# lean-dojo/ReProver

Hardware: AMD Instinct MI355X
Metric: retrieve QPS@top-100 (state encode + masked similarity top-k), ByT5-small, 130k-premise corpus (higher is better)
Workload: dtype bf16; 1 GPU; configs[1]: ByT5-small encode+retrieve, 130k premises, batch=256 states/GPU, top-100, bf16; n_premises=130000, states_per_gpu=256, k=100, state_len_mix=clip(round(LogNormal(ln 180, 0.9)), 16, 2048) bytes, index=row-sharded 1-way, bf16 unit-norm random rows, weights=random-init ByT5-small (d_model 1472, 12 layers, 6 heads, d_ff 3584)

## Files before the change

reprover_amd/csrc/rp_encoder.hip:

```cpp
#include <limits.h>

#include "rp_encoder_kernels.h"

namespace rp {

thread_local std::string g_last_error;

int g_gemm_group_m = 8;
constexpr int GEMM_VARIANT_BIG = 26, GEMM_VARIANT_O_BY_SIZE = -1;
int g_gemm_variant = GEMM_VARIANT_BIG;
int g_gemm_variant_qkv = GEMM_VARIANT_BIG;
int g_gemm_variant_wo = GEMM_VARIANT_BIG;
int g_gemm_variant_o = GEMM_VARIANT_O_BY_SIZE;
int g_gemm_small_pipe = 1;
int g_gemm_helpers = 64;
int g_gemm_persist = 9;
int g_pool_chunk = 64;
int g_gemm_edge_layout = 1;
int g_gemm_mixed = 20;
int g_gemm_mixed_bwd = 1;
int g_debug_skip_ffn = 0;
int g_gemm_skinny = 1;
int g_gemm_skinny_variant = 0;
int g_gemm_stagger_us[RP_K_COUNT] = {};

struct ProfRec {
  int cls;
  hipEvent_t a, b;
};
static bool g_prof_on = false;
static std::vector<ProfRec> g_prof_recs;
static std::vector<hipEvent_t> g_prof_pool;

static hipEvent_t prof_event() {
  if (!g_prof_pool.empty()) {
    hipEvent_t e = g_prof_pool.back();
    g_prof_pool.pop_back();
    return e;
  }
  hipEvent_t e;
  (void)hipEventCreate(&e);
  return e;
}
void prof_begin(hipStream_t stream, int kernel_class) {
  if (!g_prof_on) return;
  ProfRec r{kernel_class, prof_event(), prof_event()};
  (void)hipEventRecord(r.a, stream);
  g_prof_recs.push_back(r);
}
void prof_end(hipStream_t stream) {
  if (!g_prof_on) return;
  (void)hipEventRecord(g_prof_recs.back().b, stream);
}

}


using namespace rp;

extern "C" int32_t rp_abi_version(void) { return 7; }
extern "C" const char* rp_last_error(void) { return g_last_error.c_str(); }

namespace {
enum OptKind { OPT_PLAIN, OPT_BOOL };
struct Option {
  const char* name;
  int* var;
  int lo, hi;
  OptKind kind;
  bool (*valid)(int);
};
constexpr int ANY_LO = INT_MIN, ANY_HI = INT_MAX;
const Option g_options[] = {
    {"gemm_group_m", &g_gemm_group_m, 1, 64, OPT_PLAIN, nullptr},
    {"gemm_variant", &g_gemm_variant, ANY_LO, ANY_HI, OPT_PLAIN, gemm_variant_known},
    {"gemm_variant_qkv", &g_gemm_variant_qkv, ANY_LO, ANY_HI, OPT_PLAIN, gemm_variant_known},
    {"gemm_variant_wo", &g_gemm_variant_wo, ANY_LO, ANY_HI, OPT_PLAIN, gemm_variant_known},
    {"gemm_variant_o", &g_gemm_variant_o, ANY_LO, ANY_HI, OPT_PLAIN, gemm_variant_known},
    {"debug_skip_ffn", &g_debug_skip_ffn, ANY_LO, ANY_HI, OPT_BOOL, nullptr},
    {"gemm_skinny_variant", &g_gemm_skinny_variant, 0, 15, OPT_PLAIN, [](int v) { return v == 0 || v == 15; }},
    {"gemm_small_pipe", &g_gemm_small_pipe, ANY_LO, ANY_HI, OPT_BOOL, nullptr},
    {"pool_chunk", &g_pool_chunk, 32, 128, OPT_PLAIN, [](int v) { return v == 32 || v == 64 || v == 128; }},
    {"gemm_persist", &g_gemm_persist, ANY_LO, ANY_HI, OPT_PLAIN, nullptr},
    {"gemm_edge_layout", &g_gemm_edge_layout, ANY_LO, ANY_HI, OPT_BOOL, nullptr},
    {"gemm_mixed", &g_gemm_mixed, 0, 31, OPT_PLAIN, nullptr},
    {"gemm_mixed_bwd", &g_gemm_mixed_bwd, ANY_LO, ANY_HI, OPT_BOOL, nullptr},
    {"gemm_skinny", &g_gemm_skinny, ANY_LO, ANY_HI, OPT_BOOL, nullptr},
    {"scan_cfg", &g_scan_cfg, 0, 1, OPT_PLAIN, nullptr},
#ifdef RP_EXPERIMENTS
    {"scan_filter_cfg", &g_scan_filter_cfg, ANY_LO, ANY_HI, OPT_PLAIN, nullptr},
    {"scan_sample_cfg", &g_scan_sample_cfg, ANY_LO, ANY_HI, OPT_PLAIN, nullptr},
    {"scan_waves", &g_scan_waves, ANY_LO, ANY_HI, OPT_PLAIN, nullptr},
    {"scan_stride", &g_scan_stride, ANY_LO, ANY_HI, OPT_PLAIN, nullptr},
    {"train_dbg", &g_train_dbg, ANY_LO, ANY_HI, OPT_PLAIN, nullptr},
    {"scan_no_epilogue", &g_scan_no_epilogue, ANY_LO, ANY_HI, OPT_PLAIN, nullptr},
#endif
    {"train_wgrad_form", &g_train_wgrad_form, 0, 3, OPT_PLAIN, nullptr},
    {"scan_cap", &g_scan_cap, ANY_LO, ANY_HI, OPT_PLAIN, nullptr},
    {"scan_force_new", &g_scan_impl_force_new, ANY_LO, ANY_HI, OPT_PLAIN, nullptr},
    {"scan_small_tiles", &g_scan_small_tiles, 0, 1, OPT_PLAIN, nullptr},
    {"scan_impl", &g_scan_impl, 0, 1, OPT_PLAIN, nullptr},
};
}

extern "C" RpStatus rp_set_option(const char* name, int32_t value) {
  if (!strcmp(name, "gemm_variant_all")) {
    RP_REQUIRE(value == -1 || gemm_variant_known(value), "gemm_variant_all: tile configuration %d is not in this build", value);
    g_gemm_variant = g_gemm_variant_qkv = g_gemm_variant_wo = value < 0 ? GEMM_VARIANT_BIG : value;
    g_gemm_variant_o = value < 0 ? GEMM_VARIANT_O_BY_SIZE : value;
    return RP_OK;
  }
  if (!strcmp(name, "gemm_helpers")) {
    RP_REQUIRE(value >= 0 && value <= 248, "gemm_helpers out of range");
    g_gemm_helpers = value & ~7;
    return RP_OK;
  }
#ifdef RP_EXPERIMENTS
  if (!strncmp(name, "gemm_stagger_us_", 16)) {
    const char* which = name + 16;
    const int cls = !strcmp(which, "qkv") ? RP_K_GEMM_QKV : !strcmp(which, "o") ? RP_K_GEMM_O
                    : !strcmp(which, "wi") ? RP_K_GEMM_WI : !strcmp(which, "wo") ? RP_K_GEMM_WO : -1;
    RP_REQUIRE(cls >= 0 && value >= 0 && value <= 1000, "gemm_stagger_us: unknown GEMM or value out of range");
    g_gemm_stagger_us[cls] = value;
    return RP_OK;
  }
#endif
  for (const Option& o : g_options) {
    if (strcmp(name, o.name)) continue;
    RP_REQUIRE(value >= o.lo && value <= o.hi, "%s out of range", o.name);
    RP_REQUIRE(!o.valid || o.valid(value), "%s: %d is not one of its values in this build", o.name, value);
    *o.var = o.kind == OPT_BOOL ? value != 0 : value;
    return RP_OK;
  }
  return fail(RP_E_INVALID, "unknown option %s", name);
}

extern "C" RpStatus rp_profile_enable(int32_t on) {
  for (auto& r : g_prof_recs) {
    g_prof_pool.push_back(r.a);
    g_prof_pool.push_back(r.b);
  }
  g_prof_recs.clear();
// ... 201 lines not shown
    ProfScope ps(stream, RP_K_EMBED);
    auto launch_embed = [&](auto kern, int rows_per_wave) {
      hipLaunchKernelGGL(kern, dim3((Tp + 4 * rows_per_wave - 1) / (4 * rows_per_wave)), dim3(256), 0, stream, ids,
                         (const bf16_t*)e->embed_hi, (const uint8_t*)e->embed_lo, (const float*)e->embed_ss, w.xb,
                         reinterpret_cast<uint8_t*>(w.xlo), w.ssp, np, embed_rs ? w.rs : (float*)nullptr, 1.f / (float)D,
                         c.layer_norm_eps, T, Tp, D, c.vocab_size, t_dev);
    };
    const bool few = Tp < 8192;
    if (D <= 1536) {
      if (few) launch_embed(embed_copy_kernel<3, 1>, 1);
      else launch_embed(embed_copy_kernel<3, 4>, 4);
    } else {
      if (few) launch_embed(embed_copy_kernel<4, 1>, 1);
      else launch_embed(embed_copy_kernel<4, 4>, 4);
    }
  }
  RP_CHECK_LAUNCH();
  const dim3 att_grid(H, T / ATT_Q + batch);
  const int pc = g_pool_chunk;
  launch_worklist(cu_seqlens, batch, w.work, (int)att_grid.y, w.pwork, T / pc + batch, pc, stream);
  for (int i = 0; i < c.num_layers; ++i) {
    const LayerPacked& L = e->layers[i];
    if (!(i == 0 && embed_rs)) launch_rowscale();
    st = fused_rs ? launch_gemm<true>(w.xb, D, Tp, L.wqkv, D, 3 * inner, D,
                                      EpiStoreBf16Slots{w.qkv, 3 * inner, 3 * inner, rs_slots}, stream, RP_K_GEMM_QKV, tv, t_dev)
                  : launch_gemm(w.xb, D, Tp, L.wqkv, D, 3 * inner, D, EpiStoreBf16{w.qkv, 3 * inner, 3 * inner, rs}, stream,
                                RP_K_GEMM_QKV, tv, t_dev);
    if (st) return st;
    {
      ProfScope ps(stream, RP_K_ATTENTION);
      hipLaunchKernelGGL(attention_kernel<false>, att_grid, dim3(256), 0, stream, w.qkv, (const int4*)w.work, e->bias_tab, w.att,
                         H, e->maxd, (float*)nullptr, 0, Drop{0u, 0u, 1.f}, 0u);
    }
    if ((st = launch_gemm(w.att, inner, Tp, L.wo, inner, D, inner, EpiResid8{w.xb, w.xlo, D, D, w.ssp, np, Tp}, stream,
                          RP_K_GEMM_O, tv, t_dev)))
      return st;
    if (g_debug_skip_ffn) continue;
    launch_rowscale();
    st = fused_rs ? launch_gemm<true>(w.xb, D, Tp, L.wi, D, 2 * F, D, EpiGegluBf16Slots{w.ff, F, 2 * F, rs_slots}, stream,
                                      RP_K_GEMM_WI, tv, t_dev)
                  : launch_gemm(w.xb, D, Tp, L.wi, D, 2 * F, D, EpiGegluBf16{w.ff, F, 2 * F, rs}, stream, RP_K_GEMM_WI, tv,
                                t_dev);
    if (st) return st;
    if ((st = launch_gemm(w.ff, F, Tp, L.wo2, F, D, F, EpiResid8{w.xb, w.xlo, D, D, w.ssp, np, Tp}, stream, RP_K_GEMM_WO, tv,
                          t_dev)))
      return st;
  }
  launch_rowscale(true);
  if (hidden) {
    hipLaunchKernelGGL(hidden_out_kernel, dim3(T), dim3(256), 0, stream, w.xb, reinterpret_cast<const uint8_t*>(w.xlo), w.rs,
                       e->final_ln, hidden, D);
    RP_CHECK_LAUNCH();
    return RP_OK;
  }
  {
    ProfScope ps(stream, RP_K_POOL);
    launch_pool_partial(dim3(T / pc + batch), stream, w.xb, w.xlo, w.rs, (const int4*)w.pwork, w.pool, D, pc, e->final_ln, out,
                        out_dtype == RP_DT_BF16 ? 1 : 0, 1, true);
    launch_pool_finish(batch, stream, w.pool, e->final_ln, cu_seqlens, out, out_dtype == RP_DT_BF16 ? 1 : 0, D, pc, 1);
  }
  RP_CHECK_LAUNCH();
  return RP_OK;
}

extern "C" RpStatus rp_encode_hidden(RpEncoder* e, const int32_t* ids, const int32_t* cu_seqlens, int32_t batch, int32_t T,
                                     int32_t max_len, void* out, void* workspace, size_t workspace_bytes, void* stream_) {
  RP_REQUIRE(e && ids && cu_seqlens && out, "null argument");
  RP_REQUIRE(batch > 0 && T > 0 && max_len > 0 && max_len <= T, "batch=%d total_tokens=%d max_len=%d", batch, T,
             max_len);
  Workspace w = carve(e, T, batch, (char*)workspace);
  if (!workspace || workspace_bytes < w.bytes)
    return fail(RP_E_WORKSPACE, "workspace %zu < required %zu bytes", workspace_bytes, w.bytes);
  return encode_pass(e, ids, cu_seqlens, batch, T, nullptr, nullptr, RP_DT_BF16, w, (hipStream_t)stream_, (bf16_t*)out);
}

extern "C" RpStatus rp_encode_varlen(RpEncoder* e, const int32_t* ids, const int32_t* cu_seqlens, int32_t batch,
                                     int32_t T, int32_t max_len, void* out, int32_t out_dtype, void* workspace,
// ... 168 lines not shown
  PaddedPrep pp = carve_padded(batch, padded_len, (char*)workspace);
  Workspace w = carve(e, T_max, batch, workspace ? (char*)workspace + pp.bytes : nullptr);
  if (!workspace || workspace_bytes < pp.bytes + w.bytes)
    return fail(RP_E_WORKSPACE, "workspace %zu < required %zu bytes", workspace_bytes, pp.bytes + w.bytes);
  if (batch == 1) {
    hipLaunchKernelGGL(padded_single_kernel, dim3(1), dim3(1024), 0, stream, attention_mask, input_ids, padded_len, pp.lens,
                       pp.cu, pp.packed, meta);
  } else {
    hipLaunchKernelGGL(padded_lens_kernel, dim3(batch), dim3(256), 0, stream, attention_mask, padded_len, pp.lens);
    hipLaunchKernelGGL(padded_scan_kernel, dim3(1), dim3(1024), 0, stream, pp.lens, batch, pp.cu, meta);
    hipLaunchKernelGGL(padded_pack_kernel, dim3((padded_len + 255) / 256, batch), dim3(256), 0, stream, input_ids, pp.cu,
                       padded_len, pp.packed);
  }
  RP_CHECK_LAUNCH();
  return encode_pass(e, pp.packed, pp.cu, batch, T_max, meta , out, out_dtype, w, stream);
}

extern "C" RpStatus rp_dbg_gemm(const void* A, const void* W, void* out, int32_t M, int32_t N, int32_t K,
                                int32_t n_valid, int32_t epilogue, void* stream_) {
  hipStream_t stream = (hipStream_t)stream_;
  const bf16_t* a = (const bf16_t*)A;
  const bf16_t* w = (const bf16_t*)W;
  switch (epilogue) {
    case RP_EPI_STORE_BF16:
      return launch_gemm(a, K, M, w, K, N, K, EpiStoreBf16{(bf16_t*)out, n_valid, n_valid, RowScale{nullptr}}, stream,
                         RP_K_GEMM_QKV);
    case RP_EPI_RESID:
      RP_REQUIRE(n_valid % 8 == 0, "n_valid=%d", n_valid);
      return launch_gemm(a, K, M, w, K, N, K,
                         EpiResid{(bf16_t*)out, (bf16_t*)out + (size_t)M * n_valid, n_valid, n_valid, nullptr, 0, 0}, stream,
                         RP_K_GEMM_WO);
    case RP_EPI_RESID8:
      RP_REQUIRE(n_valid % 8 == 0, "n_valid=%d", n_valid);
      return launch_gemm(a, K, M, w, K, N, K,
                         EpiResid8{(bf16_t*)out, (bf16_t*)out + (size_t)M * n_valid, n_valid, n_valid, nullptr, 0, 0}, stream,
                         RP_K_GEMM_WO);
    case RP_EPI_GEGLU_BF16:
      return launch_gemm(a, K, M, w, K, N, K, EpiGegluBf16{(bf16_t*)out, n_valid / 2, n_valid, RowScale{nullptr}}, stream,
                         RP_K_GEMM_WI);
  }
  return fail(RP_E_INVALID, "unknown epilogue %d", epilogue);
}

extern "C" RpStatus rp_dbg_gemm_fused(const void* A, const void* W, void* out, int32_t M, int32_t N, int32_t K,
                                      int32_t n_valid, int32_t epilogue, const float* ssp_in, int32_t np_in,
                                      float inv_d, float eps, void* xb_out, float* ssp_out, int32_t np_out,
                                      void* stream_) {
  hipStream_t stream = (hipStream_t)stream_;
  const bf16_t* a = (const bf16_t*)A;
  const bf16_t* w = (const bf16_t*)W;
  float* rs_buf = nullptr;
  if (ssp_in) {
    RP_HIP(hipMalloc((void**)&rs_buf, (size_t)M * 4));
    hipLaunchKernelGGL(rowscale_kernel, dim3((M + 63) / 64), dim3(64), 0, stream, ssp_in, rs_buf, M, np_in, inv_d, eps);
  }
  const RowScale rs{rs_buf};
  struct Free {
    float* p;
    hipStream_t s;
    ~Free() {
      if (p) {
        (void)hipStreamSynchronize(s);
        (void)hipFree(p);
      }
    }
  } free_rs{rs_buf, stream};
  switch (epilogue) {
    case RP_EPI_STORE_BF16:
      return launch_gemm(a, K, M, w, K, N, K, EpiStoreBf16{(bf16_t*)out, n_valid, n_valid, rs}, stream, RP_K_GEMM_QKV);
    case RP_EPI_RESID:
      RP_REQUIRE(n_valid % 8 == 0, "n_valid=%d", n_valid);
      return launch_gemm(a, K, M, w, K, N, K,
                         EpiResid{(bf16_t*)out, (bf16_t*)out + (size_t)M * n_valid, n_valid, n_valid, ssp_out, np_out, M},
                         stream, RP_K_GEMM_WO);
    case RP_EPI_RESID8:
      RP_REQUIRE(n_valid % 8 == 0, "n_valid=%d", n_valid);
      return launch_gemm(a, K, M, w, K, N, K,
                         EpiResid8{(bf16_t*)out, (bf16_t*)out + (size_t)M * n_valid, n_valid, n_valid, ssp_out, np_out, M},
                         stream, RP_K_GEMM_WO);
    case RP_EPI_GEGLU_BF16:
      return launch_gemm(a, K, M, w, K, N, K, EpiGegluBf16{(bf16_t*)out, n_valid / 2, n_valid, rs}, stream,
                         RP_K_GEMM_WI);
  }
  return fail(RP_E_INVALID, "unknown epilogue %d", epilogue);
}

namespace rp {
__global__ __launch_bounds__(256) void mfma_probe_kernel(int mfmas, float* __restrict__ sink) {
  const uint32_t seed = (uint32_t)(blockIdx.x * 256 + threadIdx.x) * 2654435761u + 12345u;
  bf16x8 a[4], b[4];
#pragma unroll
  for (int i = 0; i < 4; ++i)
#pragma unroll
    for (int e = 0; e < 8; ++e) {
      const uint32_t h = (seed + 40503u * (uint32_t)(i * 8 + e)) * 2246822519u;
      a[i][e] = (short)(0x3f00 | (h & 0x80ff) | ((h >> 9) & 0x0080));
      b[i][e] = (short)(0x3f00 | ((h >> 16) & 0x80ff) | ((h >> 3) & 0x0080));
    }
  f32x16 acc[8];
#pragma unroll
  for (int i = 0; i < 8; ++i)
#pragma unroll
    for (int r = 0; r < 16; ++r) acc[i][r] = 0.f;
  for (int it = 0; it < mfmas; it += 32) {
#pragma unroll
    for (int rot = 0; rot < 4; ++rot)
#pragma unroll
      for (int i = 0; i < 8; ++i) acc[i] = __builtin_amdgcn_mfma_f32_32x32x16_bf16(a[i & 3], b[(i + rot) & 3], acc[i], 0, 0, 0);
  }
  float s = 0.f;
// ... 44 lines not shown
```

reprover_amd/csrc/rp_encoder_kernels.h:

```cpp
#pragma once
#include <math.h>
#include <string.h>

#include <algorithm>
#include <functional>
#include <vector>

#include "rp_gemm.h"

namespace rp {

extern int g_gemm_group_m, g_gemm_variant, g_gemm_variant_qkv, g_gemm_variant_wo, g_gemm_variant_o, g_debug_skip_ffn, g_gemm_skinny,
    g_gemm_skinny_variant, g_gemm_small_pipe, g_gemm_helpers, g_gemm_persist, g_pool_chunk, g_gemm_edge_layout, g_gemm_mixed,
    g_gemm_mixed_bwd, g_scan_waves, g_scan_small_tiles, g_scan_cfg, g_scan_impl, g_scan_filter_cfg, g_scan_sample_cfg, g_scan_stride,
    g_scan_no_epilogue, g_scan_impl_force_new, g_scan_cap, g_train_dbg, g_train_wgrad_form;
extern int g_gemm_stagger_us[RP_K_COUNT];

template <typename T>
__device__ __forceinline__ float load_as_f32(const void* p, size_t i);
template <>
__device__ __forceinline__ float load_as_f32<float>(const void* p, size_t i) {
  return reinterpret_cast<const float*>(p)[i];
}
template <>
__device__ __forceinline__ float load_as_f32<bf16_t>(const void* p, size_t i) {
  return bf2f(reinterpret_cast<const bf16_t*>(p)[i]);
}

enum PackMode { PACK_CONCAT3 = 0, PACK_GEGLU = 1, PACK_COPY = 2 };

template <typename T>
__global__ void pack_rows_kernel(bf16_t* dst, const void* s0, const void* s1, const void* s2,
                                 int rows_dst, int cols, int n, int mode, const float* colscale) {
  const int r = blockIdx.x;
  const void* src;
  int sr;
  if (mode == PACK_CONCAT3) {
    src = (r < n) ? s0 : (r < 2 * n ? s1 : s2);
    sr = r % n;
  } else if (mode == PACK_GEGLU) {
    src = ((r >> 5) & 1) ? s1 : s0;
    sr = (r >> 6) * 32 + (r & 31);
  } else {
    src = s0;
    sr = r;
  }
// ... 236 lines not shown
    for (int j = 0; j < FN; ++j) scv[j] = rs.get(n_base + j * 32 + cl);
#pragma unroll
    for (int ih = 0; ih < FM; ih += 2) {
      const int f = m_base + ih * 32 + sub * 8;
#pragma unroll
      for (int jb = 0; jb < FN; jb += 2) {
#pragma unroll
        for (int jj = 0; jj < 2 && jb + jj < FN; ++jj) {
          const float sc = scv[jb + jj];
#pragma unroll
          for (int i = 0; i < 2; ++i)
#pragma unroll
            for (int g = 0; g < 4; ++g) {
              uint2 v;
              v.x = pack_bf2(acc[ih + i][jb + jj][4 * g] * sc, acc[ih + i][jb + jj][4 * g + 1] * sc);
              v.y = pack_bf2(acc[ih + i][jb + jj][4 * g + 2] * sc, acc[ih + i][jb + jj][4 * g + 3] * sc);
              *reinterpret_cast<uint2*>(stage + (jj * 32 + cl) * EPI_ROW_BYTES + (i * 32 + 8 * g + 4 * hi) * 2) = v;
            }
        }
        const int nrows = (FN - jb >= 2) ? 64 : 32;
#pragma unroll
        for (int t0 = 0; t0 < 64; t0 += RPI) {
          const int t = t0 + rr;
          if (t < nrows) {
            const uint4 v = *reinterpret_cast<const uint4*>(stage + t * EPI_ROW_BYTES + sub * 16);
            if (f < n_valid) *reinterpret_cast<uint4*>(out + (size_t)(n_base + jb * 32 + t) * ldo + f) = v;
          }
        }
      }
    }
  }
};

template <bool SPLIT_IN, bool LO8 = false>
struct EpiResidT {
  static constexpr bool any_layout = true;
  bf16_t* __restrict__ xhi;
  bf16_t* __restrict__ xlo;
  int ldx, n_valid;
  float* __restrict__ ssp;
  int np, ssp_ld;
  const bf16_t* __restrict__ xhi_in = nullptr;
  Drop drop = {0u, 0u, 1.f};
  uint32_t drop_site = 0;
  template <int FM, int FN>
  __device__ __forceinline__ void run(f32x16 (&acc)[FM][FN], int m_base, int n_base, int lane, char* stage) {
    static_assert(FM % 2 == 0, "one statistic slot per 64 features (two row fragments)");
    const int hi = lane >> 5, cl = lane & 31;
    const int sub = lane & 7, rr = lane >> 3;
    constexpr int RB = 272;
    constexpr int NB = (FM / 2) * FN;
    constexpr int DEPTH = (FM * FN >= 16) ? 4 : 2;
    uint4 xh[DEPTH][4];
    typename std::conditional<LO8, uint2, uint4>::type xl[DEPTH][4];
    const uint8_t* xlo8 = reinterpret_cast<const uint8_t*>(xlo);
    auto fetch = [&](int b, int p) {
      const int q = b / FN, j = b % FN;
      const int f = min(m_base + q * 64 + sub * 8, n_valid - 8);
#pragma unroll
      for (int c = 0; c < 4; ++c) {
        const size_t off = (size_t)(n_base + j * 32 + c * 8 + rr) * ldx + f;
#ifdef RP_ABL_NOLOAD
        RP_ABL_NOLOAD_BODY(xh[p][c], xl[p][c], off);
#else
        if constexpr (SPLIT_IN)
          xh[p][c] = *reinterpret_cast<const uint4*>(xhi_in + off);
        else
          xh[p][c] = *reinterpret_cast<const uint4*>(xhi + off);
        if constexpr (LO8)
          xl[p][c] = *reinterpret_cast<const uint2*>(xlo8 + off);
        else
          xl[p][c] = *reinterpret_cast<const uint4*>(xlo + off);
#endif
      }
    };
#pragma unroll
    for (int b = 0; b < DEPTH - 1 && b < NB; ++b) fetch(b, b);
#pragma unroll
    for (int b = 0; b < NB; ++b) {
      const int q = b / FN, j = b % FN;
      const int f = m_base + q * 64 + sub * 8;
      const int slot = (m_base >> 6) + q;
      if (b + DEPTH - 1 < NB) fetch(b + DEPTH - 1, (b + DEPTH - 1) % DEPTH);
#pragma unroll
      for (int i = 0; i < 2; ++i)
#pragma unroll
        for (int g = 0; g < 4; ++g)
          *reinterpret_cast<float4*>(stage + cl * RB + (i * 32 + 8 * g + 4 * hi) * 4) =
              make_float4(acc[2 * q + i][j][4 * g], acc[2 * q + i][j][4 * g + 1], acc[2 * q + i][j][4 * g + 2],
                          acc[2 * q + i][j][4 * g + 3]);
#pragma unroll
      for (int c = 0; c < 4; ++c) {
        const int t = c * 8 + rr;
        float4 d0 = *reinterpret_cast<const float4*>(stage + t * RB + sub * 32);
        float4 d1 = *reinterpret_cast<const float4*>(stage + t * RB + sub * 32 + 16);
        if constexpr (SPLIT_IN) {
          if (drop.thresh) {
            const uint32_t row = (uint32_t)(n_base + j * 32 + t), c0 = (uint32_t)f;
            float m[8];
#pragma unroll
            for (int e = 0; e < 8; e += 2) drop_mul2(drop, drop_site, row, c0 + e, m[e], m[e + 1]);
            d0.x *= m[0]; d0.y *= m[1]; d0.z *= m[2]; d0.w *= m[3];
            d1.x *= m[4]; d1.y *= m[5]; d1.z *= m[6]; d1.w *= m[7];
          }
        }
        float ss = 0.f;
        if (f < n_valid) {
          const size_t off = (size_t)(n_base + j * 32 + t) * ldx + f;
          const uint4 h = xh[b % DEPTH][c];
          const auto l = xl[b % DEPTH][c];
          uint4 oh;
          typename std::conditional<LO8, uint2, uint4>::type ol;
          if constexpr (LO8) {
            x24_update8(h, l, d0, d1, oh, ol, ss);
          } else {
            hilo_update2(h.x, l.x, d0.x, d0.y, oh.x, ol.x, ss);
            hilo_update2(h.y, l.y, d0.z, d0.w, oh.y, ol.y, ss);
            hilo_update2(h.z, l.z, d1.x, d1.y, oh.z, ol.z, ss);
            hilo_update2(h.w, l.w, d1.z, d1.w, oh.w, ol.w, ss);
          }
#ifdef RP_ABL_NOSTORE
          RP_ABL_KEEP6(oh.x, oh.y, oh.z, oh.w, ol.x, ol.y);
#else
          *reinterpret_cast<uint4*>(xhi + off) = oh;
          if constexpr (LO8)
            *reinterpret_cast<uint2*>(reinterpret_cast<uint8_t*>(xlo) + off) = ol;
          else
            *reinterpret_cast<uint4*>(xlo + off) = ol;
#endif
        }
        if (ssp) {
          ss += dpp_f32<0xB1>(ss);
          ss += dpp_f32<0x4E>(ss);
          ss += dpp_f32<0x141>(ss);
          if (sub == 0 && slot < np) ssp[(size_t)slot * ssp_ld + n_base + j * 32 + t] = ss;
        }
      }
    }
  }
};

typedef EpiResidT<false> EpiResid;
typedef EpiResidT<false, true> EpiResid8;

#ifndef RP_GEGLU_PRELOAD
#define RP_GEGLU_PRELOAD 1
#endif
template <class RS>
struct EpiGegluBf16T {
  using main_layout = WaveLayout<2, 4, 4, 2>;
  bf16_t* out;
  int ldo, n_valid;
  RS rs;
  static constexpr bool preload_hook = std::is_same<RS, RowScale>::value && RP_GEGLU_PRELOAD;
  float pre[4] = {0.f, 0.f, 0.f, 0.f};
  template <int FN>
  __device__ __forceinline__ void preload(int n_base, int lane) {
    static_assert(FN <= 4, "pre[]");
#pragma unroll
    for (int j = 0; j < FN; ++j) pre[j] = rs.get(n_base + j * 32 + (lane & 31));
  }
  template <int FM, int FN, bool PRE = false>
  __device__ __forceinline__ void run(f32x16 (&acc)[FM][FN], int m_base, int n_base, int lane, char* stage) {
    static_assert(FM % 2 == 0, "gate/up fragment pairs");
    const int hi = lane >> 5, cl = lane & 31;
    constexpr int LPR = FM * 2;
    constexpr int RPI = 64 / LPR;
    static_assert(FM * 32 <= 128, "staging row");
    const int sub = lane % LPR, rr = lane / LPR;
    const int f = (m_base >> 1) + sub * 8;
    float scv[FN];
#pragma unroll
    for (int j = 0; j < FN; ++j) {
      if constexpr (PRE)
        scv[j] = pre[j];
      else
// ... 890 lines not shown
```

reprover_amd/csrc/rp_gemm.h:

```cpp
#pragma once
#include <type_traits>
#include "rp_util.h"

namespace rp {

#ifdef RP_PHASE_PROBE
#include "probes/rp_probe_hooks.h"
#else
#define RP_TS(slot) ((void)0)
#define RP_TS_PLAIN(slot) ((void)0)
#define RP_HTS(kt, which) ((void)0)
#define RP_PROBE_STAGE_FILTER(kt, half) ((void)0)
#define RP_PROBE_READS_DECL ((void)0)
#define RP_PROBE_READS_GATE ((void)0)
#define RP_PROBE_READS_PRIME(read_frags, smem) ((void)0)
#define RP_PTS_DECL ((void)0)
#define RP_PTS(v) ((void)0)
#define RP_PROBE_PERSIST_TILE_END(more) ((void)0)
#endif

__device__ __forceinline__ int mfma32_row(int r, int hi) { return (r & 3) + 8 * (r >> 2) + 4 * hi; }

template <int BM_, int BN_, int BK_, int WM_, int WN_, int NSTAGE_, int PIPE_ = 0, int FP8_ = 0, int AAUX_ = 0, int KTAIL_ = 0,
          int OCC_ = 0>
// ... 17 lines not shown
  static constexpr int A_DMA = BM / ROWS_PER_DMA / NWAVES, W_DMA = BN / ROWS_PER_DMA / NWAVES;
  static_assert(BM % (ROWS_PER_DMA * NWAVES) == 0 && BN % (ROWS_PER_DMA * NWAVES) == 0, "DMA split");
  static_assert(BK == 32 || BK == 64, "BK");
  __device__ static __forceinline__ int swz(int row) { return (BK == 32) ? ((row >> 2) & 3) : ((row >> 1) & 7); }
  __device__ static __forceinline__ int off(int row, int kc) { return row * ROW_BYTES + ((kc ^ swz(row)) << 4); }
};

template <int WM_, int WN_, int FM_, int FN_>
struct WaveLayout {
  static constexpr int WM = WM_, WN = WN_, FM = FM_, FN = FN_;
};

constexpr int EPI_ROW_BYTES = 144;
constexpr int EPI_STAGE_BYTES = 64 * EPI_ROW_BYTES;

struct GemmOperand {
  const bf16_t* ptr;
  int ld;
  int rows;
  __device__ __forceinline__ size_t row_off(int r, int kc) const { return (size_t)min(r, rows - 1) * ld + kc * 8; }
  __device__ __forceinline__ size_t k_off(int kt, int BK) const { return (size_t)kt * BK; }
};

template <class E, class = void>
struct has_prologue : std::false_type {};
template <class E>
struct has_prologue<E, std::void_t<decltype(&E::prologue)>> : std::true_type {};

template <class E, class = void>
struct has_preload : std::false_type {};
template <class E>
struct has_preload<E, std::enable_if_t<E::preload_hook>> : std::true_type {};

typedef __attribute__((address_space(3))) void* lds_ptr_t;
typedef const __attribute__((address_space(1))) void* gbl_ptr_t;

template <int N>
__device__ __forceinline__ void wait_vmcnt() {
  asm volatile("s_waitcnt vmcnt(%0)" ::"n"(N) : "memory");
}

template <class C, class Epilogue>
__device__ __forceinline__ void gemm_tile(const GemmOperand A, const GemmOperand W, int K, int tile_m,
                                          int tile_n, Epilogue& epi, char* smem) {
  constexpr int BK = C::BK, NSTAGE = C::NSTAGE, FM = C::FM, FN = C::FN;
  RP_TS_PLAIN(0);
  const int tid = threadIdx.x;
  const int lane = tid & 63;
  const int wave = __builtin_amdgcn_readfirstlane(tid >> 6);
  const int wave_row = wave / C::WN, wave_col = wave % C::WN;
  const int hi = lane >> 5;

  f32x16 acc[FM][FN];
#pragma unroll
  for (int i = 0; i < FM; ++i)
#pragma unroll
    for (int j = 0; j < FN; ++j)
#pragma unroll
      for (int r = 0; r < 16; ++r) acc[i][j][r] = 0.f;

  const bf16_t* a_src[C::A_DMA];
  const bf16_t* w_src[C::W_DMA];
#pragma unroll
  for (int d = 0; d < C::A_DMA; ++d) {
    const int row = (wave * C::A_DMA + d) * C::ROWS_PER_DMA + lane / C::SLOTS;
    const int kc = (lane % C::SLOTS) ^ C::swz(row);
    a_src[d] = A.ptr + A.row_off(tile_m * C::BM + row, kc);
  }
#pragma unroll
  for (int d = 0; d < C::W_DMA; ++d) {
    const int row = (wave * C::W_DMA + d) * C::ROWS_PER_DMA + lane / C::SLOTS;
    const int kc = (lane % C::SLOTS) ^ C::swz(row);
    w_src[d] = W.ptr + W.row_off(tile_n * C::BN + row, kc);
  }
  static_assert(C::KTAIL == 0 || (BK == 64 && C::SLOTS == 8 && C::ROWS_PER_DMA == 8 && C::FP8 != 0), "KTAIL: 128-byte e4m3 rows");
  const int nk = C::KTAIL != 0 ? (K + BK / 2) / BK : K / BK;
  const bool has_tail = C::KTAIL != 0 && nk * BK != K;
  const int fix_lane = (lane >> 2) & 1;
  auto stage = [&](int kt, int buf) {
    char* base = smem + buf * C::STAGE_BYTES;
    const int ke = kt;
    const int fix_mask = (C::KTAIL != 0 && has_tail && kt == nk - 1) ? -1 : 0;
#pragma unroll
    for (int d = 0; d < C::A_DMA; ++d) {
      const bf16_t* src = a_src[d] + A.k_off(ke, BK);
      if constexpr (C::KTAIL != 0) src += ((((fix_lane ^ (wave * C::A_DMA + d)) & 1) ? -(BK / 2) : 0) & fix_mask);
      if constexpr (C::AAUX == 2)
        __builtin_amdgcn_global_load_lds((gbl_ptr_t)src, (lds_ptr_t)(base + (wave * C::A_DMA + d) * 1024), 16, 0, 2);
      else
        __builtin_amdgcn_global_load_lds((gbl_ptr_t)src, (lds_ptr_t)(base + (wave * C::A_DMA + d) * 1024), 16, 0, 0);
    }
#pragma unroll
    for (int d = 0; d < C::W_DMA; ++d) {
      const bf16_t* src = w_src[d] + W.k_off(ke, BK);
      if constexpr (C::KTAIL != 0) src += ((((fix_lane ^ (wave * C::W_DMA + d)) & 1) ? -(BK / 2) : 0) & fix_mask);
      __builtin_amdgcn_global_load_lds((gbl_ptr_t)src, (lds_ptr_t)(base + C::A_BYTES + (wave * C::W_DMA + d) * 1024), 16, 0, 0);
    }
  };
  constexpr int DMA_PER_STAGE = C::A_DMA + C::W_DMA;

// ... 79 lines not shown
                           smem + wave * EPI_STAGE_BYTES);
  RP_TS_PLAIN(3);
}

template <class C, class Epilogue, class L = C>
__device__ __forceinline__ void gemm_tile_pipe(const GemmOperand A, const GemmOperand W, int K, int tile_m,
                                               int tile_n, Epilogue& epi, char* smem) {
  static_assert(L::WM * L::WN == C::NWAVES && L::WM * L::FM * 32 <= C::BM && L::WN * L::FN * 32 <= C::BN, "wave layout");
  constexpr int BK = C::BK, FM = L::FM, FN = L::FN, KS = C::FP8 ? C::ROW_BYTES / 64 : BK / 16;
  constexpr int RPF = C::FP8 ? 2 : 1;
  using frag_t = std::conditional_t<C::FP8 != 0, i32x8, bf16x8>;
  RP_TS(0);
  static_assert(KS % 2 == 0 && KS >= 2, "even number of k-steps (fragment double-buffer parity)");
  const int tid = threadIdx.x;
  const int lane = tid & 63;
  const int wave = __builtin_amdgcn_readfirstlane(tid >> 6);
  const int wave_row = wave / L::WN, wave_col = wave % L::WN;
  const int hi = lane >> 5;

  f32x16 acc[FM][FN];
#pragma unroll
  for (int i = 0; i < FM; ++i)
#pragma unroll
    for (int j = 0; j < FN; ++j)
#pragma unroll
      for (int r = 0; r < 16; ++r) acc[i][j][r] = 0.f;

  const bf16_t* a_src[C::A_DMA];
  const bf16_t* w_src[C::W_DMA];
#pragma unroll
  for (int d = 0; d < C::A_DMA; ++d) {
    const int row = (wave * C::A_DMA + d) * C::ROWS_PER_DMA + lane / C::SLOTS;
    const int kc = (lane % C::SLOTS) ^ C::swz(row);
    a_src[d] = A.ptr + A.row_off(tile_m * C::BM + row, kc);
  }
#pragma unroll
  for (int d = 0; d < C::W_DMA; ++d) {
    const int row = (wave * C::W_DMA + d) * C::ROWS_PER_DMA + lane / C::SLOTS;
    const int kc = (lane % C::SLOTS) ^ C::swz(row);
    w_src[d] = W.ptr + W.row_off(tile_n * C::BN + row, kc);
  }
  const int nk = C::KTAIL != 0 ? (K + BK / 2) / BK : K / BK;
  const bool has_tail = C::KTAIL != 0 && nk * BK != K;
  static_assert(C::KTAIL == 0 || (BK == 64 && C::SLOTS == 8 && C::ROWS_PER_DMA == 8), "KTAIL: 128-byte rows");
  const int fix_lane = (lane >> 2) & 1;
  if constexpr (has_prologue<Epilogue>::value) epi.prologue(smem + C::RING_BYTES, wave, lane, tile_n * C::BN);
  auto stage_half = [&](int kt, int buf, int half) {
    char* base = smem + buf * C::STAGE_BYTES;
    RP_PROBE_STAGE_FILTER(kt, half);
    const int fix_mask = (C::KTAIL != 0 && has_tail && kt == nk - 1) ? -1 : 0;
    if (half == 0) {
#pragma unroll
      for (int d = 0; d < C::A_DMA; ++d) {
        const bf16_t* src = a_src[d] + A.k_off(kt, BK);
        if constexpr (C::KTAIL != 0) src += ((((fix_lane ^ (wave * C::A_DMA + d)) & 1) ? -(BK / 2) : 0) & fix_mask);
        if constexpr (C::AAUX == 2)
          __builtin_amdgcn_global_load_lds((gbl_ptr_t)src, (lds_ptr_t)(base + (wave * C::A_DMA + d) * 1024), 16, 0, 2);
        else
          __builtin_amdgcn_global_load_lds((gbl_ptr_t)src, (lds_ptr_t)(base + (wave * C::A_DMA + d) * 1024), 16, 0, 0);
      }
    } else {
#pragma unroll
      for (int d = 0; d < C::W_DMA; ++d) {
        const bf16_t* src = w_src[d] + W.k_off(kt, BK);
        if constexpr (C::KTAIL != 0) src += ((((fix_lane ^ (wave * C::W_DMA + d)) & 1) ? -(BK / 2) : 0) & fix_mask);
        __builtin_amdgcn_global_load_lds((gbl_ptr_t)src, (lds_ptr_t)(base + C::A_BYTES + (wave * C::W_DMA + d) * 1024), 16, 0, 0);
      }
// ... 147 lines not shown
  tile_body(kt, I0(), I0());
  __syncthreads();
  RP_TS(2);

  epi.template run<FM, FN>(acc, tile_m * C::BM + wave_row * (FM * 32), tile_n * C::BN + wave_col * (FN * 32), lane,
                           smem + wave * EPI_STAGE_BYTES);
  RP_TS(3);
}

#if defined(__HIP_DEVICE_COMPILE__) && !defined(__gfx950__) && !defined(__gfx942__)
#error "gemm_tiles_persist relies on gfx942/gfx950 vmcnt semantics (loads and stores retire in order on one counter)"
#endif
constexpr int PERSIST_EPI_OFF = 64 * 1024, PERSIST_LDS_BYTES = 160 * 1024;
template <class C, bool EDGE = false, class L0 = C, class Epilogue, class NextTile>
__device__ __forceinline__ void gemm_tiles_persist(const GemmOperand A, const GemmOperand W, int K, NextTile next_tile,
                                                   Epilogue& epi, char* smem, bool edge_on = false) {
  static_assert(C::PIPE != 0 && C::FP8 == 0 && C::KTAIL == 0 && C::NSTAGE == 2 && C::STAGE_BYTES == 64 * 1024 &&
                    C::NWAVES * EPI_STAGE_BYTES <= PERSIST_LDS_BYTES - PERSIST_EPI_OFF,
                "persistent form: the pipelined 256 x 256 x 64 bf16 tile");
  constexpr int BK = C::BK, KS = BK / 16, NSTAGE = 2, DPS = C::A_DMA + C::W_DMA;
  const int tid = threadIdx.x;
  const int lane = tid & 63;
  const int wave = __builtin_amdgcn_readfirstlane(tid >> 6);
  int tile_m, tile_n;
  if (!next_tile(tile_m, tile_n)) return;

  const bf16_t* a_src[C::A_DMA];
  const bf16_t* w_src[C::W_DMA];
  auto set_src = [&](int tm, int tn) {
#pragma unroll
    for (int d = 0; d < C::A_DMA; ++d) {
      const int row = (wave * C::A_DMA + d) * C::ROWS_PER_DMA + lane / C::SLOTS;
      const int kc = (lane % C::SLOTS) ^ C::swz(row);
      a_src[d] = A.ptr + A.row_off(tm * C::BM + row, kc);
    }
#pragma unroll
    for (int d = 0; d < C::W_DMA; ++d) {
      const int row = (wave * C::W_DMA + d) * C::ROWS_PER_DMA + lane / C::SLOTS;
      const int kc = (lane % C::SLOTS) ^ C::swz(row);
      w_src[d] = W.ptr + W.row_off(tn * C::BN + row, kc);
    }
  };
  const int nk = K / BK;
  auto stage_half = [&](int kt, int buf, int half) {
    char* base = smem + buf * C::STAGE_BYTES;
    if (half == 0) {
#pragma unroll
      for (int d = 0; d < C::A_DMA; ++d)
        __builtin_amdgcn_global_load_lds((gbl_ptr_t)(a_src[d] + A.k_off(kt, BK)), (lds_ptr_t)(base + (wave * C::A_DMA + d) * 1024),
                                         16, 0, 0);
    } else {
#pragma unroll
      for (int d = 0; d < C::W_DMA; ++d)
        __builtin_amdgcn_global_load_lds((gbl_ptr_t)(w_src[d] + W.k_off(kt, BK)),
                                         (lds_ptr_t)(base + C::A_BYTES + (wave * C::W_DMA + d) * 1024), 16, 0, 0);
    }
  };
  auto stage = [&](int kt, int buf) {
    stage_half(kt, buf, 0);
    stage_half(kt, buf, 1);
  };
  using I0 = std::integral_constant<int, 0>;
  using I1 = std::integral_constant<int, 1>;
  using I2 = std::integral_constant<int, 2>;
  RP_PTS_DECL;

  auto do_tile = [&](auto layout_tag, const auto& a_off, const auto& b_off) -> bool {
// ... 176 lines not shown
```

Baseline: 8592 queries/s.

## Add register-direct residual epilogue with permuted A-row staging, off by default

Adds an optional residual-update epilogue for the O and FFN-out GEMMs. It reads and writes the hi/lo residual stream straight from the accumulator registers instead of staging through LDS, with a prefetch ring and permlane32 swaps for the row sum-of-squares. A rows are loaded in permuted order so each lane's accumulator fragment matches contiguous feature runs. The existing staged epilogue also stores one sum-of-squares per lane after the block instead of one per inner step. The direct path is gated by a new option that defaults to 0, so only the staged-epilogue store change runs by default.

After: 8574 queries/s. No clear change (-0.2%).

```diff
diff --git a/reprover_amd/csrc/rp_encoder.hip b/reprover_amd/csrc/rp_encoder.hip
--- a/reprover_amd/csrc/rp_encoder.hip
+++ b/reprover_amd/csrc/rp_encoder.hip
@@ -18,6 +18,8 @@
 int g_pool_chunk = 64;
 int g_gemm_edge_layout = 1;
 int g_gemm_mixed = 20;
+constexpr int GEMM_RESID_DIRECT_DEFAULT = 0;
+int g_gemm_resid_direct = GEMM_RESID_DIRECT_DEFAULT;
 int g_gemm_mixed_bwd = 1;
 int g_debug_skip_ffn = 0;
 int g_gemm_skinny = 1;
@@ -57,6 +59,16 @@
 
 
 using namespace rp;
+
+static RpStatus launch_gemm_resid8(const bf16_t* A, int lda, int M, const bf16_t* W, int ldw, int n_rows_w, int K,
+                                   const EpiResid8& epi, hipStream_t stream, int prof_class, int tokens_valid = 0,
+                                   const int32_t* t_dev = nullptr) {
+  if (g_gemm_resid_direct & (prof_class == RP_K_GEMM_O ? 1 : 2))
+    return launch_gemm(A, lda, M, W, ldw, n_rows_w, K,
+                       EpiResid8Direct{epi.xhi, epi.xlo, epi.ldx, epi.n_valid, epi.ssp, epi.np, epi.ssp_ld}, stream, prof_class,
+                       tokens_valid, t_dev);
+  return launch_gemm(A, lda, M, W, ldw, n_rows_w, K, epi, stream, prof_class, tokens_valid, t_dev);
+}
 
 extern "C" int32_t rp_abi_version(void) { return 7; }
 extern "C" const char* rp_last_error(void) { return g_last_error.c_str(); }
@@ -85,6 +97,7 @@
     {"gemm_edge_layout", &g_gemm_edge_layout, ANY_LO, ANY_HI, OPT_BOOL, nullptr},
     {"gemm_mixed", &g_gemm_mixed, 0, 31, OPT_PLAIN, nullptr},
     {"gemm_mixed_bwd", &g_gemm_mixed_bwd, ANY_LO, ANY_HI, OPT_BOOL, nullptr},
+    {"gemm_resid_direct", &g_gemm_resid_direct, 0, 3, OPT_PLAIN, nullptr},
     {"gemm_skinny", &g_gemm_skinny, ANY_LO, ANY_HI, OPT_BOOL, nullptr},
     {"scan_cfg", &g_scan_cfg, 0, 1, OPT_PLAIN, nullptr},
 #ifdef RP_EXPERIMENTS
@@ -108,6 +121,10 @@
     RP_REQUIRE(value == -1 || gemm_variant_known(value), "gemm_variant_all: tile configuration %d is not in this build", value);
     g_gemm_variant = g_gemm_variant_qkv = g_gemm_variant_wo = value < 0 ? GEMM_VARIANT_BIG : value;
     g_gemm_variant_o = value < 0 ? GEMM_VARIANT_O_BY_SIZE : value;
+    return RP_OK;
+  }
+  if (!strcmp(name, "gemm_resid_direct") && value == -1) {
+    g_gemm_resid_direct = GEMM_RESID_DIRECT_DEFAULT;
     return RP_OK;
   }
   if (!strcmp(name, "gemm_helpers")) {
@@ -375,7 +392,7 @@
       hipLaunchKernelGGL(attention_kernel<false>, att_grid, dim3(256), 0, stream, w.qkv, (const int4*)w.work, e->bias_tab, w.att,
                          H, e->maxd, (float*)nullptr, 0, Drop{0u, 0u, 1.f}, 0u);
     }
-    if ((st = launch_gemm(w.att, inner, Tp, L.wo, inner, D, inner, EpiResid8{w.xb, w.xlo, D, D, w.ssp, np, Tp}, stream,
+    if ((st = launch_gemm_resid8(w.att, inner, Tp, L.wo, inner, D, inner, EpiResid8{w.xb, w.xlo, D, D, w.ssp, np, Tp}, stream,
                           RP_K_GEMM_O, tv, t_dev)))
       return st;
     if (g_debug_skip_ffn) continue;
@@ -385,7 +402,7 @@
                   : launch_gemm(w.xb, D, Tp, L.wi, D, 2 * F, D, EpiGegluBf16{w.ff, F, 2 * F, rs}, stream, RP_K_GEMM_WI, tv,
                                 t_dev);
     if (st) return st;
-    if ((st = launch_gemm(w.ff, F, Tp, L.wo2, F, D, F, EpiResid8{w.xb, w.xlo, D, D, w.ssp, np, Tp}, stream, RP_K_GEMM_WO, tv,
+    if ((st = launch_gemm_resid8(w.ff, F, Tp, L.wo2, F, D, F, EpiResid8{w.xb, w.xlo, D, D, w.ssp, np, Tp}, stream, RP_K_GEMM_WO, tv,
                           t_dev)))
       return st;
   }
@@ -620,7 +637,7 @@
                          RP_K_GEMM_WO);
     case RP_EPI_RESID8:
       RP_REQUIRE(n_valid % 8 == 0, "n_valid=%d", n_valid);
-      return launch_gemm(a, K, M, w, K, N, K,
+      return launch_gemm_resid8(a, K, M, w, K, N, K,
                          EpiResid8{(bf16_t*)out, (bf16_t*)out + (size_t)M * n_valid, n_valid, n_valid, nullptr, 0, 0}, stream,
                          RP_K_GEMM_WO);
     case RP_EPI_GEGLU_BF16:
@@ -663,7 +680,7 @@
                          stream, RP_K_GEMM_WO);
     case RP_EPI_RESID8:
       RP_REQUIRE(n_valid % 8 == 0, "n_valid=%d", n_valid);
-      return launch_gemm(a, K, M, w, K, N, K,
+      return launch_gemm_resid8(a, K, M, w, K, N, K,
                          EpiResid8{(bf16_t*)out, (bf16_t*)out + (size_t)M * n_valid, n_valid, n_valid, ssp_out, np_out, M},
                          stream, RP_K_GEMM_WO);
     case RP_EPI_GEGLU_BF16:
diff --git a/reprover_amd/csrc/rp_encoder_kernels.h b/reprover_amd/csrc/rp_encoder_kernels.h
--- a/reprover_amd/csrc/rp_encoder_kernels.h
+++ b/reprover_amd/csrc/rp_encoder_kernels.h
@@ -11,7 +11,7 @@
 namespace rp {
 
 extern int g_gemm_group_m, g_gemm_variant, g_gemm_variant_qkv, g_gemm_variant_wo, g_gemm_variant_o, g_debug_skip_ffn, g_gemm_skinny,
-    g_gemm_skinny_variant, g_gemm_small_pipe, g_gemm_helpers, g_gemm_persist, g_pool_chunk, g_gemm_edge_layout, g_gemm_mixed,
+    g_gemm_skinny_variant, g_gemm_small_pipe, g_gemm_helpers, g_gemm_persist, g_pool_chunk, g_gemm_edge_layout, g_gemm_mixed, g_gemm_resid_direct,
     g_gemm_mixed_bwd, g_scan_waves, g_scan_small_tiles, g_scan_cfg, g_scan_impl, g_scan_filter_cfg, g_scan_sample_cfg, g_scan_stride,
     g_scan_no_epilogue, g_scan_impl_force_new, g_scan_cap, g_train_dbg, g_train_wgrad_form;
 extern int g_gemm_stagger_us[RP_K_COUNT];
@@ -314,8 +314,10 @@
   }
 };
 
-template <bool SPLIT_IN, bool LO8 = false>
+template <bool SPLIT_IN, bool LO8 = false, bool DIRECT = false>
 struct EpiResidT {
+  static_assert(!DIRECT || (LO8 && !SPLIT_IN), "the register path serves the inference form; the training form keeps the staged path");
+  static constexpr bool row_perm = DIRECT;
   static constexpr bool any_layout = true;
   bf16_t* __restrict__ xhi;
   bf16_t* __restrict__ xlo;
@@ -328,6 +330,10 @@
   template <int FM, int FN>
   __device__ __forceinline__ void run(f32x16 (&acc)[FM][FN], int m_base, int n_base, int lane, char* stage) {
     static_assert(FM % 2 == 0, "one statistic slot per 64 features (two row fragments)");
+    if constexpr (DIRECT) {
+      run_direct<FM, FN>(acc, m_base, n_base, lane);
+      return;
+    }
     const int hi = lane >> 5, cl = lane & 31;
     const int sub = lane & 7, rr = lane >> 3;
     constexpr int RB = 272;
@@ -371,6 +377,7 @@
           *reinterpret_cast<float4*>(stage + cl * RB + (i * 32 + 8 * g + 4 * hi) * 4) =
               make_float4(acc[2 * q + i][j][4 * g], acc[2 * q + i][j][4 * g + 1], acc[2 * q + i][j][4 * g + 2],
                           acc[2 * q + i][j][4 * g + 3]);
+      float ss_blk = 0.f;
 #pragma unroll
       for (int c = 0; c < 4; ++c) {
         const int t = c * 8 + rr;
@@ -415,8 +422,69 @@
           ss += dpp_f32<0xB1>(ss);
           ss += dpp_f32<0x4E>(ss);
           ss += dpp_f32<0x141>(ss);
-          if (sub == 0 && slot < np) ssp[(size_t)slot * ssp_ld + n_base + j * 32 + t] = ss;
+          ss_blk = (sub == c) ? ss : ss_blk;
         }
+      }
+      if (ssp && sub < 4 && slot < np) ssp[(size_t)slot * ssp_ld + n_base + j * 32 + sub * 8 + rr] = ss_blk;
+    }
+  }
+
+  template <int FM, int FN>
+  __device__ __forceinline__ void run_direct(f32x16 (&acc)[FM][FN], int m_base, int n_base, int lane) {
+    const int h = lane >> 5, cl = lane & 31;
+    constexpr int NB = (FM / 2) * FN;
+    constexpr int DEPTH = (FM * FN >= 16) ? 4 : 2;
+    uint4 xh[DEPTH][4];
+    uint2 xl[DEPTH][4];
+    uint8_t* xlo8 = reinterpret_cast<uint8_t*>(xlo);
+    auto fetch = [&](int b, int p) {
+      const int q = b / FN, j = b % FN;
+      const size_t row = (size_t)(n_base + j * 32 + cl) * ldx;
+#pragma unroll
+      for (int g = 0; g < 4; ++g) {
+        const size_t off = row + min(m_base + q * 64 + g * 16 + h * 8, n_valid - 8);
+        xh[p][g] = *reinterpret_cast<const uint4*>(xhi + off);
+        xl[p][g] = *reinterpret_cast<const uint2*>(xlo8 + off);
+      }
+    };
+    auto pair_sums = [](float a, float b) {
+      const auto r = __builtin_amdgcn_permlane32_swap(__float_as_uint(a), __float_as_uint(b), false, false);
+      return __uint_as_float(r[0]) + __uint_as_float(r[1]);
+    };
+#pragma unroll
+    for (int b = 0; b < DEPTH - 1 && b < NB; ++b) fetch(b, b);
+#pragma unroll
+    for (int b = 0; b < NB; ++b) {
+      const int q = b / FN, j = b % FN;
+      const int f0 = m_base + q * 64 + h * 8;
+      const int slot = (m_base >> 6) + q;
+      const size_t row = (size_t)(n_base + j * 32 + cl) * ldx;
+      if (b + DEPTH - 1 < NB) fetch(b + DEPTH - 1, (b + DEPTH - 1) % DEPTH);
+      uint4 oh[4];
+      uint2 ol[4];
+      float ps[4];
+#pragma unroll
+      for (int g = 0; g < 4; ++g) {
+        const f32x16& a0 = acc[2 * q][j];
+        const f32x16& a1 = acc[2 * q + 1][j];
+        float ss = 0.f;
+        x24_update8(xh[b % DEPTH][g], xl[b % DEPTH][g], make_float4(a0[4 * g], a0[4 * g + 1], a0[4 * g + 2], a0[4 * g + 3]),
+                    make_float4(a1[4 * g], a1[4 * g + 1], a1[4 * g + 2], a1[4 * g + 3]), oh[g], ol[g], ss);
+        ps[g] = (f0 + g * 16 < n_valid) ? ss : 0.f;
+      }
+#pragma unroll
+      for (int g = 0; g < 4; ++g)
+        if (f0 + g * 16 < n_valid) {
+          const size_t off = row + f0 + g * 16;
+          *reinterpret_cast<uint4*>(xhi + off) = oh[g];
+          *reinterpret_cast<uint2*>(xlo8 + off) = ol[g];
+        }
+      if (ssp) {
+        const float u = pair_sums(ps[0], ps[1]);
+        const float v = pair_sums(ps[2], ps[3]);
+        const float w = pair_sums(u, v);
+        const float s = pair_sums(w, w);
+        if (h == 0 && slot < np) ssp[(size_t)slot * ssp_ld + n_base + j * 32 + cl] = s;
       }
     }
   }
@@ -424,6 +492,7 @@
 
 typedef EpiResidT<false> EpiResid;
 typedef EpiResidT<false, true> EpiResid8;
+typedef EpiResidT<false, true, true> EpiResid8Direct;
 
 #ifndef RP_GEGLU_PRELOAD
 #define RP_GEGLU_PRELOAD 1
diff --git a/reprover_amd/csrc/rp_gemm.h b/reprover_amd/csrc/rp_gemm.h
--- a/reprover_amd/csrc/rp_gemm.h
+++ b/reprover_amd/csrc/rp_gemm.h
@@ -73,6 +73,21 @@
 template <class E>
 struct has_preload<E, std::enable_if_t<E::preload_hook>> : std::true_type {};
 
+template <class E, class = void>
+struct has_row_perm : std::false_type {};
+template <class E>
+struct has_row_perm<E, std::enable_if_t<E::row_perm>> : std::true_type {};
+__device__ __forceinline__ int resid_row_perm(int row) {
+  return (row & ~63) | (((row >> 3) & 3) << 4) | (((row >> 2) & 1) << 3) | (((row >> 5) & 1) << 2) | (row & 3);
+}
+template <class E>
+__device__ __forceinline__ int m_src_row(int row) {
+  if constexpr (has_row_perm<E>::value)
+    return resid_row_perm(row);
+  else
+    return row;
+}
+
 typedef __attribute__((address_space(3))) void* lds_ptr_t;
 typedef const __attribute__((address_space(1))) void* gbl_ptr_t;
 
@@ -106,7 +121,7 @@
   for (int d = 0; d < C::A_DMA; ++d) {
     const int row = (wave * C::A_DMA + d) * C::ROWS_PER_DMA + lane / C::SLOTS;
     const int kc = (lane % C::SLOTS) ^ C::swz(row);
-    a_src[d] = A.ptr + A.row_off(tile_m * C::BM + row, kc);
+    a_src[d] = A.ptr + A.row_off(tile_m * C::BM + m_src_row<Epilogue>(row), kc);
   }
 #pragma unroll
   for (int d = 0; d < C::W_DMA; ++d) {
@@ -252,7 +267,7 @@
   for (int d = 0; d < C::A_DMA; ++d) {
     const int row = (wave * C::A_DMA + d) * C::ROWS_PER_DMA + lane / C::SLOTS;
     const int kc = (lane % C::SLOTS) ^ C::swz(row);
-    a_src[d] = A.ptr + A.row_off(tile_m * C::BM + row, kc);
+    a_src[d] = A.ptr + A.row_off(tile_m * C::BM + m_src_row<Epilogue>(row), kc);
   }
 #pragma unroll
   for (int d = 0; d < C::W_DMA; ++d) {
@@ -466,7 +481,7 @@
     for (int d = 0; d < C::A_DMA; ++d) {
       const int row = (wave * C::A_DMA + d) * C::ROWS_PER_DMA + lane / C::SLOTS;
       const int kc = (lane % C::SLOTS) ^ C::swz(row);
-      a_src[d] = A.ptr + A.row_off(tm * C::BM + row, kc);
+      a_src[d] = A.ptr + A.row_off(tm * C::BM + m_src_row<Epilogue>(row), kc);
     }
 #pragma unroll
     for (int d = 0; d < C::W_DMA; ++d) {
```
